# mbrzus/Cross-Modality-Minipig-Gan

Measured on AMD Instinct MI355X. Metric: T1->T2 256x256 slices/sec (G+D step), higher is better.
Workload: dtype f32

## Files before the change

cross-modality-minipig-gan_amd/_lib.py:

```python
from __future__ import annotations

import ctypes as C
import os

_HERE = os.path.dirname(os.path.abspath(__file__))
LIB_PATH = os.environ.get("MPGAN_LIB_PATH") or os.path.join(_HERE, "libmpgan_hip.so")
_lib = None


class ConvGeomC(C.Structure):
    _fields_ = [("n", C.c_int32), ("in_dhw", C.c_int32 * 3), ("out_dhw", C.c_int32 * 3),
                ("cin", C.c_int32), ("cout", C.c_int32), ("k", C.c_int32 * 3),
                ("stride", C.c_int32 * 3), ("pad", C.c_int32 * 3), ("transposed", C.c_int32),
                ("flags", C.c_int32), ("min_blocks", C.c_int32)]


class PeerTapsC(C.Structure):
    _fields_ = [("z_peer", C.c_void_p), ("ld_peer", C.c_int32), ("scale_peer", C.c_void_p),
                ("shift_peer", C.c_void_p), ("coef", C.c_void_p)]


class PeerTapsBF16C(C.Structure):
    _fields_ = [("z_peer", C.c_void_p), ("ld_peer", C.c_int32), ("scale_peer", C.c_void_p),
                ("shift_peer", C.c_void_p), ("coef", C.c_void_p)]
# ... 41 lines not shown
    "mpgan_conv_backward_data_stats_bf16": (_I, [_G, _P, _I, _P, _P, _I, _P, _I, _P, _P, _P, _P, _F, _P, _P]),
    "mpgan_conv_backward_data_stats": (_I, [_G, _P, _I, _P, _P, _I, _P, _I, _P, _P, _P, _P, _I, _F, _P, _P]),
    "mpgan_conv_wgrad_workspace": (_L, [_G]),
    "mpgan_conv_backward_weight": (_I, [_G, _P, _I, _PR, _P, _I, _P, _P, _F, _P, _L, _P]),
    "mpgan_conv_wgrad_kernel_name": (_I, [_G, _I, _I, C.c_char_p, _I]),
    "mpgan_pack_weights": (_I, [_P, _P, _P, _I, _L, _P]),
    "mpgan_stats_chunks": (_I, [_L, _I]),
    "mpgan_channel_stats": (_I, [_P, _I, _I, _L, _I, _P, _P]),
    "mpgan_norm_finalize": (_I, [_P, _I, _I, _I, _L, _I, _P, _P, _F, _F, _P, _P, _P, _P, _P, _P, _P, _P]),
    "mpgan_norm_finalize_strided": (_I, [_P, _I, _I, _I, _I, _L, _I, _P, _P, _F, _F, _P, _P, _P, _P, _P, _P, _P, _P]),
    "mpgan_norm_from_running": (_I, [_P, _P, _P, _P, _F, _I, _P, _P, _P, _P, _P]),
    "mpgan_norm_from_running_multi": (_I, [_P, _I, _P]),
    "mpgan_epi_vectors_multi": (_I, [_P, _I, _P]),
    "mpgan_conv_forward_act": (_I, [_G, _P, _I, _P, _P, _P, _P, _P, _I, _I, _P, _I, _P]),
    "mpgan_norm_act_add": (_I, [_P, _I, _PR, _P, _I, _PR, _I, _L, _I, _I, _P, _I, _P]),
    "mpgan_norm_bwd_reduce": (_I, [_P, _I, _P, _I, _PR, _P, _P, C.POINTER(PeerTapsC), _I, _L, _I, _P, _P]),
    "mpgan_tap_l1_partials": (_I, []),
    "mpgan_tap_l1": (_I, [_P, _I, _PR, _P, _I, _PR, _L, _I, _P, _P, _P]),
    "mpgan_conv_splitk_workspace": (_L, [_G]),
    "mpgan_conv_forward_splitk": (_I, [_G, _P, _I, _P, _P, _PR, _P, _L, _P, _I, _P]),
    "mpgan_sigmoid_forward": (_I, [_P, _I, _P, _P]),
    "mpgan_norm_bwd_finalize": (_I, [_P, _I, _I, _I, _L, _I, _P, _P, _P, _P, _P, _P]),
    "mpgan_norm_bwd_apply": (_I, [_P, _I, _P, _I, _PR, _P, _P, _P, _P, C.POINTER(PeerTapsC), _I, _L, _I, _P, _I, _P]),
    "mpgan_reduce_partials": (_I, [_P, _I, _I, _I, _P, _F, _P]),
    "mpgan_add_tanh": (_I, [_P, _P, _L, _I, _P, _P]),
    "mpgan_tanh_backward": (_I, [_P, _P, _L, _P, _P]),
    "mpgan_axpby": (_I, [_P, _F, _P, _F, _L, _P, _P]),
    "mpgan_copy_slice": (_I, [_P, _I, _P, _I, _L, _I, _I, _P]),
    "mpgan_linear1_partials": (_I, [_I]),
    "mpgan_linear1_forward": (_I, [_P, _PR, _I, _L, _I, _P, _P, _P, _P, _P, _P]),
    "mpgan_bce_forward": (_I, [_P, _P, _I, _P, _P]),
    "mpgan_bce_backward": (_I, [_P, _P, _I, _P, _P, _P]),
    "mpgan_sigmoid_backward": (_I, [_P, _P, _I, _P, _P]),
    "mpgan_scale_by_device_scalar": (_I, [_P, _P, _L, _P, _P]),
    "mpgan_weighted_sum": (_I, [_P, _P, _I, _P, _P]),
    "mpgan_debug_stamps": (_I, [_P, _L, _L]),
    "mpgan_debug_stamps_used": (_L, []),
    "mpgan_debug_clock_khz": (_I, []),
    "mpgan_linear1_backward": (_I, [_P, _PR, _I, _L, _I, _P, _P, _P, _P, _P, _F, _P]),
    "mpgan_sigmoid_bce": (_I, [_P, _I, _F, _F, _P, _P, _P, _P]),
    "mpgan_l1_partials": (_I, []),
    "mpgan_l1_loss": (_I, [_P, _P, _L, _F, _P, _P, _P, _P]),
    "mpgan_metric_partials": (_I, []),
    "mpgan_rescale_minmax": (_I, [_P, _L, _F, _F, _I, _P, _P, _P, _P]),
    "mpgan_image_errors": (_I, [_P, _P, _L, _F, _P, _P, _P]),
    "mpgan_percentile_workspace": (_L, []),
# ... 76 lines not shown
```

cross-modality-minipig-gan_amd/csrc/norm_ops.hip:

```cpp
#include "mpgan_common.h"
#include "norm_fold.h"

namespace mpgan {

static inline int stats_chunks_host(long pixels_per_sample, int C = 0) {
  long rows = 256;
  if (C >= 4 && C % 4 == 0) {
    long R = 256 / (C / 4);
    if (R < 1) R = 1;
    rows = 4 * R;
    if (rows > 256) rows = 256;
    if (rows < 16) rows = 16;
  }
  long c = pixels_per_sample / rows;
  if (c < 1) c = 1;
  if (c > 256) c = 256;
  return (int)c;
}

template <int V>
struct Vec;
template <>
struct Vec<4> {
  using T = float4;
// ... 514 lines not shown
      if (!ok[u]) continue;
      const long row = (long)n * P + pix0 + u * stride;
      float o[V];
#pragma unroll
      for (int e = 0; e < V; ++e) {
        const float y = zv[u][e] * sc[e] + sh[e];
        const float zh = (zv[u][e] - mu[e]) * is[e];
        float ga = gv[u][e], gy_extra = 0.f, dz_extra = 0.f;
        if (pr.coef) {
          const float yp = zp[u][e] * psc[e] + psh[e];
          const float ap = (leaky && yp < 0.f) ? yp * slope : yp;
          const float a = (leaky && y < 0.f) ? y * slope : y;
          ga -= ca * sgn(ap - a);
          gy_extra = -cy * sgn(yp - y);
          dz_extra = -cz * sgn(zp[u][e] - zv[u][e]);
        }
        const float gy = ((leaky && y < 0.f) ? ga * slope : ga) + gy_extra;
        o[e] = sc[e] * (gy - k1[e] - zh * k2[e]) + dz_extra;
      }
      Vec<V>::store(dz + row * lddz + c, o);
    }
  }
  (void)rows;
}

__global__ __launch_bounds__(256) void tap_l1_kernel(const float* __restrict__ za, int lda, Pro pa,
                                                     const float* __restrict__ zb, int ldb, Pro pb, long rows, int C,
                                                     float* __restrict__ partials) {
  __shared__ float sh[3][4];
  const float sa = pro_slope(pa), sb = pro_slope(pb);
  float s0 = 0.f, s1 = 0.f, s2 = 0.f;
  const long total = rows * C;
  for (long i = (long)blockIdx.x * blockDim.x + threadIdx.x; i < total; i += (long)gridDim.x * blockDim.x) {
    const long row = i / C;
    const int c = (int)(i - row * C);
    const float z1 = za[row * lda + c], z2 = zb[row * ldb + c];
    const float y1 = z1 * pa.scale[c] + pa.shift[c], y2 = z2 * pb.scale[c] + pb.shift[c];
    const float a1 = act_apply(y1, pa.act, sa), a2 = act_apply(y2, pb.act, sb);
    s0 += fabsf(z1 - z2);
    s1 += fabsf(y1 - y2);
    s2 += fabsf(a1 - a2);
  }
  s0 = wave_sum(s0); s1 = wave_sum(s1); s2 = wave_sum(s2);
  const int lane = threadIdx.x & 63, w = threadIdx.x >> 6;
  if (lane == 0) { sh[0][w] = s0; sh[1][w] = s1; sh[2][w] = s2; }
  __syncthreads();
// ... 226 lines not shown
                      ldg >= c && ldz >= c && lddz >= c,
                  "norm_bwd_apply: bad argument");
  const bool vec = (c % 4 == 0) && (ldz % 4 == 0) && (ldg % 4 == 0) && (lddz % 4 == 0) && aligned16(z) &&
                   aligned16(g) && aligned16(dz);
  const long rows = (long)n * P;
  Pro pp = make_pro(p);
  Peer pe = make_peer(peer);
  const int CGa = vec ? c / 4 : c;
  MPGAN_UNSUPPORTED(CGa > 256, "norm_bwd_apply: C=%d too wide", c);
  const int Ra = 256 / CGa;
  long gxa = (P + 4L * Ra - 1) / (4L * Ra);
  const long capa = 4096 / n > 1 ? 4096 / n : 1;
  if (gxa > capa) gxa = capa;
  dim3 grida((unsigned)gxa, (unsigned)n);
  if (vec)
    hipLaunchKernelGGL(norm_bwd_apply_kernel<4>, grida, dim3(256), 0, (hipStream_t)stream, g, ldg, z, ldz, pp, mean,
                       invstd, c1, c2, pe, rows, (long)P, c, dz, lddz);
  else
    hipLaunchKernelGGL(norm_bwd_apply_kernel<1>, grida, dim3(256), 0, (hipStream_t)stream, g, ldg, z, ldz, pp, mean,
                       invstd, c1, c2, pe, rows, (long)P, c, dz, lddz);
  return check_launch("norm_bwd_apply");
}

extern "C" int mpgan_reduce_partials(const float* partials, int32_t rows, int32_t row_stride, int32_t c, float* out,
                                     float beta, void* stream) {
  MPGAN_CHECK_ARG(partials && out && rows > 0 && c > 0 && row_stride >= c, "reduce_partials: bad argument");
  hipLaunchKernelGGL(reduce_partials_kernel, dim3((c + 3) / 4), dim3(256), 0, (hipStream_t)stream, partials, rows,
                     row_stride, c, out, beta);
  return check_launch("reduce_partials");
}

extern "C" int mpgan_copy_slice(const float* src, int32_t lds_, float* dst, int32_t ldd, int64_t pixels, int32_t c,
                                int32_t accumulate, void* stream) {
  MPGAN_CHECK_ARG(src && dst && pixels > 0 && c > 0 && lds_ >= c && ldd >= c, "copy_slice: bad argument");
  const bool vec = (c % 4 == 0) && (lds_ % 4 == 0) && (ldd % 4 == 0) && aligned16(src) && aligned16(dst);
  if (vec)
    hipLaunchKernelGGL(copy_slice_kernel<4>, dim3(ew_blocks(pixels * (c / 4))), dim3(256), 0, (hipStream_t)stream, src,
                       lds_, dst, ldd, (long)pixels, c, accumulate);
  else
    hipLaunchKernelGGL(copy_slice_kernel<1>, dim3(ew_blocks(pixels * c)), dim3(256), 0, (hipStream_t)stream, src, lds_,
                       dst, ldd, (long)pixels, c, accumulate);
  return check_launch("copy_slice");
}

__global__ void norm_from_running_kernel(const float* __restrict__ gamma, const float* __restrict__ beta,
                                         const float* __restrict__ rm, const float* __restrict__ rv, float eps, int c,
// ... 104 lines not shown
```

cross-modality-minipig-gan_amd/engine.py:

```python
from __future__ import annotations

import ctypes as C
import dataclasses
import math
import os
from typing import List, Optional, Sequence, Tuple

import torch
import torch.nn as nn

from . import ops
from ._lib import lib
from .ops import ACT_LEAKY, ACT_NONE, ConvGeom, Prologue


class KernelProbe:

    def __init__(self, want=None, detail=False, min_flops=0.0):
        self.want = want
        self.detail = detail
        self.min_flops = min_flops
        self.samples = []

    def summary(self):
# ... 438 lines not shown
                 C.byref(pc) if pc is not None else None, _p(resid), _ld(resid), int(tanh), _p(stats), y.data_ptr(),
                 _ld(y), keep=(gc, pc, x, wp, bias, y, resid, pro), desc=_gdesc(g), tag=tag, lane=lane)
        return
    assert stats is None or stats_acc is None
    prog.add("conv_forward_fold", lib().mpgan_conv_forward_fold, C.byref(gc), x.data_ptr(), _ld(x), wp.data_ptr(),
             _p(bias), C.byref(pc) if pc is not None else None, C.byref(fold) if fold is not None else None, _p(resid),
             _ld(resid), int(tanh), _p(stats), _p(stats_acc), ops.ACC_REPLICAS if stats_acc is not None else 0,
             y.data_ptr(), _ld(y), keep=(gc, pc, fold, x, wp, bias, y, resid, pro, stats_acc), desc=_gdesc(g), tag=tag,
             lane=lane)


def emit_conv_dgrad(prog, g: ConvGeom, dy, wp_bwd, dx, resid=None):
    ops._check_in_out(g, dx, dy, "plan conv_backward_data")
    gc = g.c()
    prog.add("conv_backward_data", lib().mpgan_conv_backward_data, C.byref(gc), dy.data_ptr(), _ld(dy),
             wp_bwd.data_ptr(), _p(resid), _ld(resid), dx.data_ptr(), _ld(dx), keep=(gc, dy, wp_bwd, dx, resid),
             desc=_gdesc(g), tag=("dgrad:" + gather_kernel_name(g, True, False), 2.0 * conv_macs(g), conv_bytes(g)))


_FUSE_BWD_STATS = not os.environ.get("MPGAN_DBG_NO_FUSE_BWD_STATS")
_FUSE_BWD_STATS_BF16 = bool(os.environ.get("MPGAN_FUSE_BWD_STATS_BF16"))


def emit_conv_dgrad_stats(prog, g: ConvGeom, dy, wp_bwd, dx, z, nb: "NormBuf", slope: float, partials) -> int:
    rows = ops.conv_bwd_stats_rows(g) if _FUSE_BWD_STATS and not nb.instance else 0
    if not rows or partials.numel() < rows * 3 * g.cin:
        emit_conv_dgrad(prog, g, dy, wp_bwd, dx)
        return 0
    ops._check_in_out(g, dx, dy, "plan conv_backward_data_stats")
    gc = g.c()
    prog.add("conv_backward_data", lib().mpgan_conv_backward_data_stats, C.byref(gc), dy.data_ptr(), _ld(dy),
             wp_bwd.data_ptr(), dx.data_ptr(), _ld(dx), z.data_ptr(), _ld(z), nb.scale.data_ptr(), nb.shift.data_ptr(),
             nb.mean.data_ptr(), nb.invstd.data_ptr(), ACT_LEAKY, float(slope), partials.data_ptr(),
             keep=(gc, dy, wp_bwd, dx, z, nb, partials), desc=_gdesc(g),
             tag=("dgrad:" + gather_kernel_name(g, True, False), 2.0 * conv_macs(g), conv_bytes(g)))
    return rows


def emit_conv_wgrad(prog, g: ConvGeom, x, dy, dw, ws, pro=None, dbias=None, lane=0):
    ops._check_in_out(g, x, dy, "plan conv_backward_weight")
    gc = g.c()
    pc = pro.c() if pro is not None else None
    need = ops.conv_wgrad_workspace(g)
    assert ws.numel() * 4 >= need, "wgrad workspace too small"
    prog.add("conv_backward_weight", lib().mpgan_conv_backward_weight, C.byref(gc), x.data_ptr(), _ld(x),
             C.byref(pc) if pc is not None else None, dy.data_ptr(), _ld(dy), dw.data_ptr(), _p(dbias), 1.0,
# ... 164 lines not shown
                 tag=_thin_cin1_tag(g, x))
        return
    prog.add("conv_forward_act_bf16", lib().mpgan_conv_forward_act_bf16, C.byref(gc), x.data_ptr(), g.cin, wp.data_ptr(),
             vec[0].data_ptr(), vec[1].data_ptr(), vec[2].data_ptr(), None, y.data_ptr(), g.cout,
             int(y.dtype == torch.float32), keep=(gc, x, wp, y, vec, norm_mod, act_mod, bias), desc=_gdesc(g),
             tag=(_bf16_kernel_name(g, False), 2.0 * conv_macs(g), conv_bytes(g, 2)))


def emit_norm_act_add(prog, z, pz, r, pr, out, tanh=False, fold=None):
    n, P, ldz = ops._cl(z, "norm_act_add z")
    assert out.shape == z.shape and (r is None or r.shape == z.shape)
    pzc = pz.c() if pz is not None else None
    prc = pr.c() if pr is not None else None
    if fold is None:
        prog.add("norm_act_add", lib().mpgan_norm_act_add, z.data_ptr(), ldz, C.byref(pzc) if pzc else None, _p(r),
                 _ld(r), C.byref(prc) if prc else None, n, P, z.shape[-1], int(tanh), out.data_ptr(), _ld(out),
                 keep=(z, pzc, pz, r, prc, pr, out), desc=f"C{z.shape[-1]} n{n} P{P}")
        return
    prog.add("norm_act_add_fold", lib().mpgan_norm_act_add_fold, z.data_ptr(), ldz, C.byref(pzc), C.byref(fold), _p(r),
             _ld(r), C.byref(prc) if prc else None, n, P, z.shape[-1], int(tanh), out.data_ptr(), _ld(out),
             keep=(z, pzc, pz, fold, r, prc, pr, out))


def emit_norm_bwd(prog, g, z, nb: NormBuf, pro: Prologue, dz, partials, dgamma, dbeta, dslope, peer=None, reduced_rows=0):
    n, P, ldz = ops._cl(z, "norm_bwd z")
    assert g.shape == z.shape and dz.shape == z.shape
    c = z.shape[-1]
    chunks = ops.stats_chunks(P, c)
    assert partials.numel() >= n * chunks * (3 * c + 1)
    L = lib()
    pc = pro.c()
    pe = peer.c() if peer is not None else None
    pe_ref = C.byref(pe) if pe is not None else None
    if reduced_rows:
        assert peer is None and not nb.instance and partials.numel() >= reduced_rows * 3 * c
        assert dslope is None, "fused norm-backward rows cannot feed a slope gradient"
        prog.add("norm_bwd_finalize", L.mpgan_norm_bwd_finalize, partials.data_ptr(), 1, reduced_rows, c, n * P, 0,
                 _p(dgamma), _p(dbeta), _p(dslope), nb.c1.data_ptr(), nb.c2.data_ptr(), keep=(dgamma, dbeta, dslope))
        prog.add("norm_bwd_apply", L.mpgan_norm_bwd_apply, g.data_ptr(), _ld(g), z.data_ptr(), ldz, C.byref(pc),
                 nb.mean.data_ptr(), nb.invstd.data_ptr(), nb.c1.data_ptr(), nb.c2.data_ptr(), pe_ref, n, P, c,
                 dz.data_ptr(), _ld(dz), keep=(dz, g, z, pc, pro, nb, partials), desc=f"C{c} n{n} P{P}")
        return
    prog.add("norm_bwd_reduce", L.mpgan_norm_bwd_reduce, g.data_ptr(), _ld(g), z.data_ptr(), ldz, C.byref(pc),
             nb.mean.data_ptr(), nb.invstd.data_ptr(), pe_ref, n, P, c, partials.data_ptr(),
             keep=(g, z, pc, pro, nb, partials, pe, peer), desc=f"C{c} n{n} P{P}")
    prog.add("norm_bwd_finalize", L.mpgan_norm_bwd_finalize, partials.data_ptr(), n, chunks, c, P, int(nb.instance),
             _p(dgamma), _p(dbeta), _p(dslope), nb.c1.data_ptr(), nb.c2.data_ptr(), keep=(dgamma, dbeta, dslope),
             desc=f"C{c} rows{n * chunks}")
    prog.add("norm_bwd_apply", L.mpgan_norm_bwd_apply, g.data_ptr(), _ld(g), z.data_ptr(), ldz, C.byref(pc),
             nb.mean.data_ptr(), nb.invstd.data_ptr(), nb.c1.data_ptr(), nb.c2.data_ptr(), pe_ref, n, P, c,
             dz.data_ptr(), _ld(dz), keep=(dz,), desc=f"C{c} n{n} P{P}")


def _bf16_kernel_name(g: ConvGeom, backward_data: bool) -> str:
    gc = g.c()
    return kernel_label(lib().mpgan_conv_kernel_name_bf16, C.byref(gc), int(backward_data))


def _bf16_wgrad_kernel_name(g: ConvGeom) -> str:
    gc = g.c()
    return "wgrad_bf16_wide_kernel" if lib().mpgan_conv_wgrad_variant_bf16(C.byref(gc)) == 1 else "wgrad_bf16_kernel<8>"


def _thin_cin1_tag(g: ConvGeom, x):
    return ("thin_cin1_full_kernel<16, true>", 2.0 * conv_macs(g), conv_bytes(g, 2) + 2 * x.numel())


def _rows(g: ConvGeom) -> int:
    return g.n * math.prod(g.out_dhw)


class PacksBF16:

    def __init__(self, recs, dev):
# ... 130 lines not shown
    def __exit__(self, *a):
        _GEOM_DEFAULTS.clear()
        _GEOM_DEFAULTS.update(self.saved)
        return False


def conv_geom_of(mod, n, in_dhw, dims) -> ConvGeom:
    tr = isinstance(mod, (nn.ConvTranspose2d, nn.ConvTranspose3d))
    k, s, p = _t3(mod.kernel_size, dims, 1), _t3(mod.stride, dims, 1), _t3(mod.padding, dims, 0)
    op = _t3(mod.output_padding, dims, 0) if tr else (0, 0, 0)
    return ConvGeom(n, tuple(in_dhw), mod.in_channels, mod.out_channels, k, s, p, tr, op, **_GEOM_DEFAULTS)


class Scratch:

    def __init__(self, dev):
        self.dev = dev
        self.partials_need = 0
        self.ws_need = 0
        self.partials = None
        self.ws = None

    def want_partials(self, n, P, c):
        self.partials_need = max(self.partials_need, (n * ops.stats_chunks(P, c) + 32) * (3 * c + 1) + c)

    def want_ws(self, g: ConvGeom):
        self.ws_need = max(self.ws_need, ops.conv_wgrad_workspace(g) // 4)
        rows = max(ops.conv_stats_rows(g, code) for code in (0, 1, 2))
        self.partials_need = max(self.partials_need, (rows + 32) * 2 * g.cout)

    def want_bf16_layer(self, g: ConvGeom, fused_rows=0):
        c, rows = g.cout, _rows(g)
        fwd_rows = (rows + 255) // 256 if g.cin == 1 else ops.conv_stats_rows_bf16(g)
        bwd_rows = max(ops.norm_bwd_rows_bf16(rows, c), fused_rows)
        self.partials_need = max(self.partials_need, (fwd_rows + 32) * 2 * c, (bwd_rows * 4 + 1) * c)
        ws = ops.conv_wgrad_workspace_bf16dy(g) if g.cin == 1 else ops.conv_wgrad_workspace_bf16(g)
        self.ws_need = max(self.ws_need, ws // 4)

    def alloc(self):
        self.partials = torch.empty(max(self.partials_need, 4), device=self.dev)
        self.ws = torch.empty(max(self.ws_need, 4), device=self.dev)


class _RU:

    def __init__(self, ru):
        self.units = []
# ... 255 lines not shown
            return

        own_mark, wait_mark = self._marks
        bw = Program()
        if wait_mark is not None:
            b.wait(wait_mark)
        G = a["gbufs"]
        gv = store.grad_view
        g_out, g_x = G["g_out"], G["g_x"]
        for l in range(0, L - 1):
            u = up_state[l]
            pt = prelu_pro(u["nbt"], u["AT"])
            g_u = g_out if l == 0 else G["gcat"][l - 1][..., chans[l - 1]:]
            if "zu" in u:
                dzu, gta = G["dzu"][l], G["gta"][l]
                emit_norm_bwd(b, g_u, u["zu"], u["nbu"], prelu_pro(u["nbu"], u["AU"]), dzu, part,
                              gv(u["NU"].weight), gv(u["NU"].bias), gv(u["AU"].weight))
                emit_conv_wgrad(bw, u["gu"], u["zt"], dzu, gv(u["cu"].weight), ws, pro=pt, dbias=gv(u["cu"].bias), lane=1)
                emit_conv_dgrad(b, u["gu"], dzu, wpb(R(u["cu"])), gta, resid=g_u)
            else:
                gta = G["gta"][l]
                emit_conv_wgrad(bw, u["gu"], u["ua"], g_u, gv(u["cu"].weight), ws, dbias=gv(u["cu"].bias), lane=1)
                emit_conv_dgrad(b, u["gu"], g_u, wpb(R(u["cu"])), gta, resid=g_u)
            emit_norm_bwd(b, gta, u["zt"], u["nbt"], pt, gta, part, gv(u["NT"].weight), gv(u["NT"].bias),
                          gv(u["AT"].weight))
            emit_bias_grad(b, gta, gv(u["ct"].bias), part)
            emit_conv_wgrad(bw, u["gt"], cats[l], gta, gv(u["ct"].weight), ws, lane=1)
            emit_conv_dgrad(b, u["gt"], gta, wpb(R(u["ct"])), G["gcat"][l])
        gcat_last = G["gcat"][L - 2]
        g_b = gcat_last[..., bt["cb_in"]:]
        gd_last = gcat_last[..., :bt["cb_in"]]
        d_last = cats[L - 2][..., :bt["cb_in"]]
        dzb1, gab0 = G["dzb1"], G["gab0"]
        emit_norm_bwd(b, g_b, bt["zb1"], bt["nbb1"], prelu_pro(bt["nbb1"], bt["BA1"]), dzb1, part,
                      gv(bt["BN1"].weight), gv(bt["BN1"].bias), gv(bt["BA1"].weight))
        emit_conv_wgrad(bw, bt["gb1"], bt["zb0"], dzb1, gv(bt["bc1"].weight), ws, pro=prelu_pro(bt["nbb0"], bt["BA0"]),
                        dbias=gv(bt["bc1"].bias), lane=1)
        emit_conv_dgrad(b, bt["gb1"], dzb1, wpb(R(bt["bc1"])), gab0)
        emit_norm_bwd(b, gab0, bt["zb0"], bt["nbb0"], prelu_pro(bt["nbb0"], bt["BA0"]), gab0, part,
                      gv(bt["BN0"].weight), gv(bt["BN0"].bias), gv(bt["BA0"].weight))
        emit_conv_wgrad(bw, bt["gb0"], d_last, gab0, gv(bt["bc0"].weight), ws, dbias=gv(bt["bc0"].bias), lane=1)
        emit_conv_dgrad(b, bt["gb0"], gab0, wpb(R(bt["bc0"])), gd_last, resid=gd_last)
        if bt["res"] is not None:
            emit_conv_wgrad(bw, bt["gbr"], d_last, g_b, gv(bt["res"].weight), ws, dbias=gv(bt["res"].bias), lane=1)
            emit_conv_dgrad(b, bt["gbr"], g_b, wpb(R(bt["res"])), gd_last, resid=gd_last)
        else:
            emit_norm_act_add(b, g_b, None, gd_last, None, gd_last)
        for l in range(L - 2, -1, -1):
            s = down_state[l]
            (cv0, N0, A0), (cv1, N1, A1) = s["ru"].units
            g_d = G["gcat"][l][..., :s["c"]]
            dz1, ga0 = G["dz1"][l], G["ga0"][l]
            emit_norm_bwd(b, g_d, s["z1"], s["nb1"], prelu_pro(s["nb1"], A1), dz1, part, gv(N1.weight), gv(N1.bias),
                          gv(A1.weight))
            emit_conv_wgrad(bw, s["g1"], s["z0"], dz1, gv(cv1.weight), ws, pro=prelu_pro(s["nb0"], A0),
                            dbias=gv(cv1.bias), lane=1)
            emit_conv_dgrad(b, s["g1"], dz1, wpb(R(cv1)), ga0)
            emit_norm_bwd(b, ga0, s["z0"], s["nb0"], prelu_pro(s["nb0"], A0), ga0, part, gv(N0.weight), gv(N0.bias),
                          gv(A0.weight))
            emit_conv_wgrad(bw, s["g0"], s["xin"], ga0, gv(cv0.weight), ws, dbias=gv(cv0.bias), lane=1)
            emit_conv_wgrad(bw, s["gr"], s["xin"], g_d, gv(s["ru"].res.weight), ws, dbias=gv(s["ru"].res.bias), lane=1)
            if l > 0:
                tgt = G["gcat"][l - 1][..., :chans[l - 1]]
                emit_conv_dgrad(b, s["g0"], ga0, wpb(R(cv0)), tgt, resid=tgt)
                emit_conv_dgrad(b, s["gr"], g_d, wpb(R(s["ru"].res)), tgt, resid=tgt)
            elif g_x is not None:
                emit_conv_dgrad(b, s["g0"], ga0, wpb(R(cv0)), g_x)
                emit_conv_dgrad(b, s["gr"], g_d, wpb(R(s["ru"].res)), g_x, resid=g_x)
        b.extend(bw)
        if own_mark is not None:
# ... 706 lines not shown
```

cross-modality-minipig-gan_amd/ops.py:

```python
from __future__ import annotations

import ctypes as C
import dataclasses
from dataclasses import dataclass
from typing import Optional, Sequence, Tuple

import torch

from ._lib import ConvGeomC, NormFoldC, PeerTapsBF16C, PeerTapsC, PrologueC, check, lib

ACT_NONE = 0
ACT_LEAKY = 1


def _stream() -> int:
    return torch.cuda.current_stream().cuda_stream


def _ptr(t: Optional[torch.Tensor]) -> Optional[int]:
    return None if t is None else t.data_ptr()


def _clx(t: torch.Tensor, dtype, what: str) -> Tuple[int, int, int]:
    if t.dim() != 5 or t.dtype != dtype or not t.is_cuda:
        raise ValueError(f"{what}: need a CUDA {dtype} (N,D,H,W,C) tensor, got {tuple(t.shape)} {t.dtype} {t.device}")
    n, d, h, w, c = t.shape
    st = t.stride()
    ld = st[3] if w > 1 else (st[2] if h > 1 else (st[1] if d > 1 else (st[0] if n > 1 else c)))
# ... 289 lines not shown
        raise ValueError("norm_bwd_reduce: partials too small (need n*chunks*(3*c + 1) floats)")
    check(lib().mpgan_norm_bwd_reduce(g.data_ptr(), ldg, z.data_ptr(), ldz, _pro(p), mean.data_ptr(),
                                      invstd.data_ptr(), _peer(peer), n, P, c, partials.data_ptr(), _stream()),
          "norm_bwd_reduce")


def norm_bwd_finalize(partials, n, chunks, c, P, instance, dgamma, dbeta, dslope, c1, c2):
    check(lib().mpgan_norm_bwd_finalize(partials.data_ptr(), n, chunks, c, P, int(instance), _ptr(dgamma), _ptr(dbeta),
                                        _ptr(dslope), c1.data_ptr(), c2.data_ptr(), _stream()), "norm_bwd_finalize")


def norm_bwd_apply(g, z, p: Prologue, mean, invstd, c1, c2, dz, peer: Optional[PeerTaps] = None):
    n, P, ldz = _cl(z, "norm_bwd_apply z")
    _, _, ldg = _cl(g, "norm_bwd_apply g")
    _, _, lddz = _cl(dz, "norm_bwd_apply dz")
    if g.shape != z.shape or dz.shape != z.shape:
        raise ValueError("norm_bwd_apply: shape mismatch")
    check(lib().mpgan_norm_bwd_apply(g.data_ptr(), ldg, z.data_ptr(), ldz, _pro(p), mean.data_ptr(),
                                     invstd.data_ptr(), c1.data_ptr(), c2.data_ptr(), _peer(peer), n, P, z.shape[-1],
                                     dz.data_ptr(), lddz, _stream()), "norm_bwd_apply")
    return dz


def tap_l1_partials() -> int:
    return int(lib().mpgan_tap_l1_partials())


def tap_l1(za, pa: Prologue, zb, pb: Prologue, partials, out3):
    n, P, lda = _cl(za, "tap_l1 a")
    _, _, ldb = _cl(zb, "tap_l1 b")
    if za.shape != zb.shape:
        raise ValueError("tap_l1: shape mismatch")
    check(lib().mpgan_tap_l1(za.data_ptr(), lda, _pro(pa), zb.data_ptr(), ldb, _pro(pb), n * P, za.shape[-1],
                             partials.data_ptr(), out3.data_ptr(), _stream()), "tap_l1")
    return out3


def conv_splitk_workspace(g: ConvGeom) -> int:
    gc = g.c()
    return int(lib().mpgan_conv_splitk_workspace(C.byref(gc)))


def conv_forward_splitk(g: ConvGeom, x, w_packed, bias, y, workspace, *, pro: Optional[Prologue] = None):
    _check_in_out(g, x, y, "conv_forward_splitk")
    _, _, ldx = _cl(x, "conv_forward_splitk x")
    _, _, ldy = _cl(y, "conv_forward_splitk y")
# ... 478 lines not shown
```

include/mpgan_hip.h:

```cpp
#ifndef MPGAN_HIP_H
#define MPGAN_HIP_H

#include <stdint.h>

#ifdef __cplusplus
extern "C" {
#endif

#define MPGAN_OK 0
#define MPGAN_ERR_INVALID -1
#define MPGAN_ERR_UNSUPPORTED -2
#define MPGAN_ERR_HIP -3

#define MPGAN_ACT_NONE 0
#define MPGAN_ACT_LEAKY 1

const char* mpgan_last_error(void);
int mpgan_abi_version(void);

typedef struct {
  int32_t n;
  int32_t in_dhw[3];
  int32_t out_dhw[3];
  int32_t cin, cout;
// ... 99 lines not shown

int mpgan_epi_vectors_multi(const int64_t* table, int32_t n_layers, void* stream);

int mpgan_norm_act_add(const float* z, int32_t ldz, const mpgan_prologue* pz,
                       const float* r, int32_t ldr, const mpgan_prologue* pr,
                       int32_t n, int64_t pixels_per_sample, int32_t c, int32_t tanh_out,
                       float* out, int32_t ldo, void* stream);

int mpgan_norm_bwd_reduce(const float* g, int32_t ldg, const float* z, int32_t ldz,
                          const mpgan_prologue* p, const float* mean, const float* invstd,
                          const mpgan_peer_taps* peer ,
                          int32_t n, int64_t pixels_per_sample, int32_t c,
                          float* partials, void* stream);
int mpgan_norm_bwd_finalize(const float* partials, int32_t n, int32_t chunks, int32_t c,
                            int64_t pixels_per_sample, int32_t instance,
                            float* dgamma, float* dbeta, float* dslope,
                            float* c1, float* c2, void* stream);
int mpgan_norm_bwd_apply(const float* g, int32_t ldg, const float* z, int32_t ldz,
                         const mpgan_prologue* p, const float* mean, const float* invstd,
                         const float* c1, const float* c2,
                         const mpgan_peer_taps* peer ,
                         int32_t n, int64_t pixels_per_sample, int32_t c,
                         float* dz, int32_t lddz, void* stream);

int mpgan_reduce_partials(const float* partials, int32_t rows, int32_t row_stride, int32_t c,
                          float* out, float beta, void* stream);

int mpgan_add_tanh(const float* a, const float* b, int64_t numel, int32_t apply_tanh,
                   float* y, void* stream);
int mpgan_tanh_backward(const float* g, const float* y, int64_t numel, float* dx, void* stream);
int mpgan_axpby(const float* a, float alpha, const float* b, float beta, int64_t numel,
                float* y, void* stream);
int mpgan_copy_slice(const float* src, int32_t lds, float* dst, int32_t ldd, int64_t pixels,
                     int32_t c, int32_t accumulate, void* stream);

int32_t mpgan_linear1_partials(int32_t n);
int mpgan_linear1_forward(const float* z, const mpgan_prologue* p, int32_t n,
                          int64_t pixels_per_sample, int32_t c, const float* w_perm,
                          const float* bias, float* partials, float* logit, float* prob ,
                          void* stream);
int mpgan_linear1_backward(const float* z, const mpgan_prologue* p, int32_t n,
                           int64_t pixels_per_sample, int32_t c, const float* w_perm,
                           const float* dlogit, float* g_a, float* dw, float* dbias,
                           float beta, void* stream);

int mpgan_sigmoid_bce(const float* logit, int32_t n, float target, float loss_scale,
// ... 200 lines not shown
```

Measured before the change: 294.6.

## Add folded BatchNorm backward kernels with fused bias grad and early wgrad flush

Adds an opt-in BatchNorm backward path. Reduction partials are folded per block and then finalized inside the apply kernel, which removes the separate finalize launch. The apply kernel also emits column sums so the conv bias gradient can be reduced without another pass over the gradient. Separately, the accumulated weight-gradient lane is flushed into the main backward program before the down-path loop by default. This changes the ordering and overlap of wgrad with dgrad work. The fold path is env-gated; the early wgrad reorder is active and may reduce or worsen overlap.

```diff
diff --git a/cross-modality-minipig-gan_amd/_lib.py b/cross-modality-minipig-gan_amd/_lib.py
--- a/cross-modality-minipig-gan_amd/_lib.py
+++ b/cross-modality-minipig-gan_amd/_lib.py
@@ -87,6 +87,9 @@
     "mpgan_sigmoid_forward": (_I, [_P, _I, _P, _P]),
     "mpgan_norm_bwd_finalize": (_I, [_P, _I, _I, _I, _L, _I, _P, _P, _P, _P, _P, _P]),
     "mpgan_norm_bwd_apply": (_I, [_P, _I, _P, _I, _PR, _P, _P, _P, _P, C.POINTER(PeerTapsC), _I, _L, _I, _P, _I, _P]),
+    "mpgan_norm_bwd_fold_rows": (_I, [_I, _L, _I, _P, _P, _P]),
+    "mpgan_norm_bwd_reduce_fold": (_I, [_P, _I, _P, _I, _PR, _P, _P, _I, _L, _I, _P, _P]),
+    "mpgan_norm_bwd_apply_fold": (_I, [_P, _I, _P, _I, _PR, _P, _P, _P, _I, _L, _I, _P, _P, _P, _P, _P, _P, _I, _P, _P]),
     "mpgan_reduce_partials": (_I, [_P, _I, _I, _I, _P, _F, _P]),
     "mpgan_add_tanh": (_I, [_P, _P, _L, _I, _P, _P]),
     "mpgan_tanh_backward": (_I, [_P, _P, _L, _P, _P]),
diff --git a/cross-modality-minipig-gan_amd/csrc/norm_ops.hip b/cross-modality-minipig-gan_amd/csrc/norm_ops.hip
--- a/cross-modality-minipig-gan_amd/csrc/norm_ops.hip
+++ b/cross-modality-minipig-gan_amd/csrc/norm_ops.hip
@@ -560,6 +560,225 @@
     }
   }
   (void)rows;
+}
+
+struct FoldLayout {
+  int rows, groups, Cg, adopt;
+};
+
+static inline FoldLayout fold_layout(int n, long P, int C) {
+  FoldLayout L;
+  L.groups = 1;
+  L.Cg = C;
+  if (C % 4 == 0)
+    while (L.Cg > 32 && L.Cg % 8 == 0) { L.Cg /= 2; L.groups *= 2; }
+  const long T = (long)n * P;
+  const int cgq = (C % 4 == 0) ? L.Cg / 4 : L.Cg;
+  const long R = cgq >= 256 ? 1 : 256 / cgq;
+  long rows = T / (4 * R);
+  const long cap = (48L * 1024 / 4) / (3L * C + L.groups);
+  if (rows > cap) rows = cap;
+  if (rows > 256) rows = 256;
+  if (rows < 1) rows = 1;
+  L.rows = (int)rows;
+  const bool vec_c = C % 4 == 0;
+  L.adopt = (C <= 128 && cap >= 1 && (vec_c || T * C <= (1L << 20))) ? 1 : 0;
+  return L;
+}
+
+static inline int fold_apply_blocks(int n, long P, int C) {
+  const int CG = (C % 4 == 0) ? C / 4 : C;
+  const long R = 256 / CG;
+  long b = ((long)n * P + 8 * R - 1) / (8 * R);
+  if (b > 256) b = 256;
+  if (b < 1) b = 1;
+  return (int)b;
+}
+
+template <int V>
+__global__ __launch_bounds__(256) void norm_bwd_reduce_fold_kernel(const float* __restrict__ gr, int ldg,
+                                                                   const float* __restrict__ z, int ldz, Pro p,
+                                                                   const float* __restrict__ mean,
+                                                                   const float* __restrict__ invstd, long T, int Cg,
+                                                                   float* __restrict__ partials) {
+  extern __shared__ float red[];
+  const float slope = pro_slope(p);
+  const bool leaky = p.act == MPGAN_ACT_LEAKY;
+  const int CGq = Cg / V, R = 256 / CGq;
+  const int tid = threadIdx.x;
+  const int q = tid % CGq, r = tid / CGq;
+  const int rows = gridDim.x, rb = blockIdx.x, grp = blockIdx.y;
+  const int cl = q * V, c = grp * Cg + cl;
+  const long per = (T + rows - 1) / rows;
+  const long beg = (long)rb * per;
+  const long end = beg + per < T ? beg + per : T;
+  float acc[3][V];
+#pragma unroll
+  for (int a = 0; a < 3; ++a)
+#pragma unroll
+    for (int e = 0; e < V; ++e) acc[a][e] = 0.f;
+  if (r < R) {
+    float sc[V], sh[V], mu[V], is[V];
+#pragma unroll
+    for (int e = 0; e < V; ++e) {
+      sc[e] = p.scale[c + e]; sh[e] = p.shift[c + e]; mu[e] = mean[c + e]; is[e] = invstd[c + e];
+    }
+    for (long pix0 = beg + r; pix0 < end; pix0 += 4L * R) {
+      float zv[4][V], gv[4][V];
+      bool ok[4];
+#pragma unroll
+      for (int u = 0; u < 4; ++u) {
+        const long pix = pix0 + (long)u * R;
+        ok[u] = pix < end;
+        const long row = ok[u] ? pix : pix0;
+        Vec<V>::load(z + row * ldz + c, zv[u]);
+        Vec<V>::load(gr + row * ldg + c, gv[u]);
+      }
+#pragma unroll
+      for (int u = 0; u < 4; ++u) {
+        if (!ok[u]) continue;
+#pragma unroll
+        for (int e = 0; e < V; ++e) {
+          const float y = zv[u][e] * sc[e] + sh[e];
+          const float zh = (zv[u][e] - mu[e]) * is[e];
+          const float ga = gv[u][e];
+          const bool neg = leaky && y < 0.f;
+          const float gy = neg ? ga * slope : ga;
+          acc[0][e] += gy;
+          acc[1][e] += gy * zh;
+          acc[2][e] += neg ? ga * y : 0.f;
+        }
+      }
+    }
+#pragma unroll
+    for (int a = 0; a < 3; ++a)
+#pragma unroll
+      for (int e = 0; e < V; ++e) red[(r * 3 + a) * Cg + cl + e] = acc[a][e];
+  }
+  __syncthreads();
+  const long rowi = (long)grp * rows + rb;
+  fold_rows(red, R, 3 * Cg, partials + rowi * 3 * Cg);
+  __syncthreads();
+  if (tid < 64) {
+    float t = 0.f;
+    for (int j = tid; j < Cg; j += 64) t += red[2 * Cg + j];
+    t = wave_sum(t);
+    if (tid == 0) partials[(long)gridDim.x * gridDim.y * 3 * Cg + rowi] = t;
+  }
+}
+
+template <int V>
+__global__ __launch_bounds__(256) void norm_bwd_apply_fold_kernel(const float* gr, int ldg, const float* __restrict__ z,
+                                                                  int ldz, Pro p, const float* __restrict__ mean,
+                                                                  const float* __restrict__ invstd,
+                                                                  const float* __restrict__ partials, int frows,
+                                                                  int groups, int Cg, double cnt, float* dgamma,
+                                                                  float* dbeta, float* dslope, float* c1, float* c2,
+                                                                  long T, int C, float* dz, int lddz,
+                                                                  float* __restrict__ colsum) {
+  __shared__ double fsum[256];
+  __shared__ float k1s[128], k2s[128];
+  __shared__ float cs[256 * V];
+  const int tid = threadIdx.x;
+  {
+    const int W = 2 * C;
+    int G = 1;
+    while (2 * G * W <= 256) G *= 2;
+    const int i = tid % W, gq = tid / W;
+    if (gq < G) {
+      const int qn = i / C, ch = i - qn * C;
+      const int grp = ch / Cg, cc = ch - grp * Cg;
+      const float* __restrict__ col = partials + ((long)grp * frows * 3 + qn) * Cg + cc;
+      double s = 0.0;
+      for (int r = gq; r < frows; r += 4 * G) {
+        float v[4];
+#pragma unroll
+        for (int u = 0; u < 4; ++u) {
+          const int rr = r + u * G;
+          v[u] = rr < frows ? col[(long)rr * 3 * Cg] : 0.f;
+        }
+#pragma unroll
+        for (int u = 0; u < 4; ++u) s += (double)v[u];
+      }
+      fsum[gq * W + i] = s;
+    }
+    __syncthreads();
+    for (int h = G >> 1; h > 0; h >>= 1) {
+      if (gq < h) fsum[gq * W + i] += fsum[(gq + h) * W + i];
+      __syncthreads();
+    }
+    if (tid < W) {
+      const double tot = fsum[tid];
+      const float k = (float)(tot / cnt);
+      if (tid < C) {
+        k1s[tid] = k;
+        if (blockIdx.x == 0) {
+          c1[tid] = k;
+          if (dbeta) dbeta[tid] += (float)tot;
+        }
+      } else {
+        k2s[tid - C] = k;
+        if (blockIdx.x == 0) {
+          c2[tid - C] = k;
+          if (dgamma) dgamma[tid - C] += (float)tot;
+        }
+      }
+    }
+    if (dslope && blockIdx.x == 0) slope_grad_block(partials + (long)frows * 3 * C, groups * frows, 0, dslope);
+    __syncthreads();
+  }
+  const int CG = C / V, R = 256 / CG;
+  const int q = tid % CG, r = tid / CG;
+  const int c = q * V;
+  const bool active = r < R;
+  float csum[V];
+#pragma unroll
+  for (int e = 0; e < V; ++e) csum[e] = 0.f;
+  if (active) {
+    const float slope = pro_slope(p);
+    const bool leaky = p.act == MPGAN_ACT_LEAKY;
+    float sc[V], sh[V], mu[V], is[V], k1[V], k2[V];
+#pragma unroll
+    for (int e = 0; e < V; ++e) {
+      sc[e] = p.scale[c + e]; sh[e] = p.shift[c + e]; mu[e] = mean[c + e]; is[e] = invstd[c + e];
+      k1[e] = k1s[c + e]; k2[e] = k2s[c + e];
+    }
+    const long stride = (long)gridDim.x * R;
+    for (long pix0 = (long)blockIdx.x * R + r; pix0 < T; pix0 += 4 * stride) {
+      float zv[4][V], gv[4][V];
+      bool ok[4];
+#pragma unroll
+      for (int u = 0; u < 4; ++u) {
+        const long pix = pix0 + u * stride;
+        ok[u] = pix < T;
+        const long row = ok[u] ? pix : pix0;
+        Vec<V>::load(z + row * ldz + c, zv[u]);
+        Vec<V>::load(gr + row * ldg + c, gv[u]);
+      }
+#pragma unroll
+      for (int u = 0; u < 4; ++u) {
+        if (!ok[u]) continue;
+        const long row = pix0 + u * stride;
+        float o[V];
+#pragma unroll
+        for (int e = 0; e < V; ++e) {
+          const float y = zv[u][e] * sc[e] + sh[e];
+          const float zh = (zv[u][e] - mu[e]) * is[e];
+          const float ga = gv[u][e];
+          const float gy = (leaky && y < 0.f) ? ga * slope : ga;
+          o[e] = sc[e] * (gy - k1[e] - zh * k2[e]);
+          csum[e] += o[e];
+        }
+        Vec<V>::store(dz + row * lddz + c, o);
+      }
+    }
+  }
+  if (!colsum) return;
+  if (active)
+#pragma unroll
+    for (int e = 0; e < V; ++e) cs[r * C + c + e] = csum[e];
+  __syncthreads();
+  fold_rows(cs, R, C, colsum + (long)blockIdx.x * C);
 }
 
 __global__ __launch_bounds__(256) void tap_l1_kernel(const float* __restrict__ za, int lda, Pro pa,
@@ -832,6 +1051,67 @@
   return check_launch("norm_bwd_apply");
 }
 
+extern "C" int32_t mpgan_norm_bwd_fold_rows(int32_t n, int64_t P, int32_t c, int32_t* groups, int32_t* apply_blocks,
+                                            int32_t* adopt) {
+  if (n <= 0 || P <= 0 || c <= 0) return 0;
+  const FoldLayout L = fold_layout(n, (long)P, c);
+  if (groups) *groups = L.groups;
+  if (apply_blocks) *apply_blocks = fold_apply_blocks(n, (long)P, c);
+  if (adopt) *adopt = L.adopt;
+  return L.rows;
+}
+
+extern "C" int mpgan_norm_bwd_reduce_fold(const float* g, int32_t ldg, const float* z, int32_t ldz,
+                                          const mpgan_prologue* p, const float* mean, const float* invstd, int32_t n,
+                                          int64_t P, int32_t c, float* partials, void* stream) {
+  MPGAN_CHECK_ARG(g && z && p && p->scale && mean && invstd && partials && n > 0 && P > 0 && c > 0 && ldg >= c &&
+                      ldz >= c,
+                  "norm_bwd_reduce_fold: bad argument");
+  MPGAN_UNSUPPORTED(p->n_stride != 0, "norm_bwd_reduce_fold: BatchNorm layers only (per-sample statistics given)");
+  const FoldLayout L = fold_layout(n, (long)P, c);
+  MPGAN_UNSUPPORTED(c > 128, "norm_bwd_reduce_fold: C=%d too wide", c);
+  const bool vec = (c % 4 == 0) && (ldz % 4 == 0) && (ldg % 4 == 0) && aligned16(z) && aligned16(g);
+  const int R = 256 / (vec ? L.Cg / 4 : L.Cg);
+  dim3 grid(L.rows, L.groups);
+  const size_t smem = (size_t)R * 3 * L.Cg * sizeof(float);
+  Pro pp = make_pro(p);
+  const long T = (long)n * P;
+  if (vec)
+    hipLaunchKernelGGL(norm_bwd_reduce_fold_kernel<4>, grid, dim3(256), smem, (hipStream_t)stream, g, ldg, z, ldz, pp,
+                       mean, invstd, T, L.Cg, partials);
+  else
+    hipLaunchKernelGGL(norm_bwd_reduce_fold_kernel<1>, grid, dim3(256), smem, (hipStream_t)stream, g, ldg, z, ldz, pp,
+                       mean, invstd, T, L.Cg, partials);
+  return check_launch("norm_bwd_reduce_fold");
+}
+
+extern "C" int mpgan_norm_bwd_apply_fold(const float* g, int32_t ldg, const float* z, int32_t ldz,
+                                         const mpgan_prologue* p, const float* mean, const float* invstd,
+                                         const float* partials, int32_t n, int64_t P, int32_t c, float* dgamma,
+                                         float* dbeta, float* dslope, float* c1, float* c2, float* dz, int32_t lddz,
+                                         float* colsum_partials, void* stream) {
+  MPGAN_CHECK_ARG(g && z && p && p->scale && mean && invstd && partials && c1 && c2 && dz && n > 0 && P > 0 && c > 0 &&
+                      ldg >= c && ldz >= c && lddz >= c,
+                  "norm_bwd_apply_fold: bad argument");
+  MPGAN_UNSUPPORTED(p->n_stride != 0, "norm_bwd_apply_fold: BatchNorm layers only (per-sample statistics given)");
+  const FoldLayout L = fold_layout(n, (long)P, c);
+  MPGAN_UNSUPPORTED(c > 128, "norm_bwd_apply_fold: C=%d too wide", c);
+  const bool vec = (c % 4 == 0) && (ldz % 4 == 0) && (ldg % 4 == 0) && (lddz % 4 == 0) && aligned16(z) &&
+                   aligned16(g) && aligned16(dz);
+  Pro pp = make_pro(p);
+  const long T = (long)n * P;
+  dim3 grida((unsigned)fold_apply_blocks(n, (long)P, c));
+  if (vec)
+    hipLaunchKernelGGL(norm_bwd_apply_fold_kernel<4>, grida, dim3(256), 0, (hipStream_t)stream, g, ldg, z, ldz, pp,
+                       mean, invstd, partials, L.rows, L.groups, L.Cg, (double)T, dgamma, dbeta, dslope, c1, c2, T, c,
+                       dz, lddz, colsum_partials);
+  else
+    hipLaunchKernelGGL(norm_bwd_apply_fold_kernel<1>, grida, dim3(256), 0, (hipStream_t)stream, g, ldg, z, ldz, pp,
+                       mean, invstd, partials, L.rows, L.groups, L.Cg, (double)T, dgamma, dbeta, dslope, c1, c2, T, c,
+                       dz, lddz, colsum_partials);
+  return check_launch("norm_bwd_apply_fold");
+}
+
 extern "C" int mpgan_reduce_partials(const float* partials, int32_t rows, int32_t row_stride, int32_t c, float* out,
                                      float beta, void* stream) {
   MPGAN_CHECK_ARG(partials && out && rows > 0 && c > 0 && row_stride >= c, "reduce_partials: bad argument");
diff --git a/cross-modality-minipig-gan_amd/engine.py b/cross-modality-minipig-gan_amd/engine.py
--- a/cross-modality-minipig-gan_amd/engine.py
+++ b/cross-modality-minipig-gan_amd/engine.py
@@ -484,6 +484,10 @@
 _FUSE_BWD_STATS_BF16 = bool(os.environ.get("MPGAN_FUSE_BWD_STATS_BF16"))
 
 
+_NORM_BWD_FOLD = bool(os.environ.get("MPGAN_NORM_BWD_FOLD"))
+_EARLY_WGRAD = not os.environ.get("MPGAN_DBG_LATE_WGRAD")
+
+
 def emit_conv_dgrad_stats(prog, g: ConvGeom, dy, wp_bwd, dx, z, nb: "NormBuf", slope: float, partials) -> int:
     rows = ops.conv_bwd_stats_rows(g) if _FUSE_BWD_STATS and not nb.instance else 0
     if not rows or partials.numel() < rows * 3 * g.cin:
@@ -694,10 +698,29 @@
              keep=(z, pzc, pz, fold, r, prc, pr, out))
 
 
-def emit_norm_bwd(prog, g, z, nb: NormBuf, pro: Prologue, dz, partials, dgamma, dbeta, dslope, peer=None, reduced_rows=0):
+def norm_bwd_folds(n, P, c, nb: "NormBuf", peer=None, reduced_rows=0) -> bool:
+    return bool(_NORM_BWD_FOLD and peer is None and not nb.instance and not reduced_rows
+                and ops.norm_bwd_fold_layout(n, P, c).adopt)
+
+
+def emit_norm_bwd(prog, g, z, nb: NormBuf, pro: Prologue, dz, partials, dgamma, dbeta, dslope, peer=None, reduced_rows=0,
+                  colsum=None) -> bool:
     n, P, ldz = ops._cl(z, "norm_bwd z")
     assert g.shape == z.shape and dz.shape == z.shape
     c = z.shape[-1]
+    if norm_bwd_folds(n, P, c, nb, peer, reduced_rows):
+        lay = ops.norm_bwd_fold_layout(n, P, c)
+        assert partials.numel() >= lay.partials(c) and not pro.n_stride
+        assert colsum is None or colsum.numel() >= lay.apply_blocks * c
+        L, pc = lib(), pro.c()
+        prog.add("norm_bwd_reduce_fold", L.mpgan_norm_bwd_reduce_fold, g.data_ptr(), _ld(g), z.data_ptr(), ldz,
+                 C.byref(pc), nb.mean.data_ptr(), nb.invstd.data_ptr(), n, P, c, partials.data_ptr(),
+                 keep=(g, z, pc, pro, nb, partials), desc=f"C{c} n{n} P{P}")
+        prog.add("norm_bwd_apply_fold", L.mpgan_norm_bwd_apply_fold, g.data_ptr(), _ld(g), z.data_ptr(), ldz,
+                 C.byref(pc), nb.mean.data_ptr(), nb.invstd.data_ptr(), partials.data_ptr(), n, P, c, _p(dgamma),
+                 _p(dbeta), _p(dslope), nb.c1.data_ptr(), nb.c2.data_ptr(), dz.data_ptr(), _ld(dz), _p(colsum),
+                 keep=(dz, dgamma, dbeta, dslope, colsum), desc=f"C{c} n{n} P{P} rows{lay.rows}x{lay.groups}")
+        return colsum is not None
     chunks = ops.stats_chunks(P, c)
     assert partials.numel() >= n * chunks * (3 * c + 1)
     L = lib()
@@ -712,7 +735,7 @@
         prog.add("norm_bwd_apply", L.mpgan_norm_bwd_apply, g.data_ptr(), _ld(g), z.data_ptr(), ldz, C.byref(pc),
                  nb.mean.data_ptr(), nb.invstd.data_ptr(), nb.c1.data_ptr(), nb.c2.data_ptr(), pe_ref, n, P, c,
                  dz.data_ptr(), _ld(dz), keep=(dz, g, z, pc, pro, nb, partials), desc=f"C{c} n{n} P{P}")
-        return
+        return False
     prog.add("norm_bwd_reduce", L.mpgan_norm_bwd_reduce, g.data_ptr(), _ld(g), z.data_ptr(), ldz, C.byref(pc),
              nb.mean.data_ptr(), nb.invstd.data_ptr(), pe_ref, n, P, c, partials.data_ptr(),
              keep=(g, z, pc, pro, nb, partials, pe, peer), desc=f"C{c} n{n} P{P}")
@@ -722,6 +745,7 @@
     prog.add("norm_bwd_apply", L.mpgan_norm_bwd_apply, g.data_ptr(), _ld(g), z.data_ptr(), ldz, C.byref(pc),
              nb.mean.data_ptr(), nb.invstd.data_ptr(), nb.c1.data_ptr(), nb.c2.data_ptr(), pe_ref, n, P, c,
              dz.data_ptr(), _ld(dz), keep=(dz,), desc=f"C{c} n{n} P{P}")
+    return False
 
 
 def _bf16_kernel_name(g: ConvGeom, backward_data: bool) -> str:
@@ -898,7 +922,8 @@
         self.ws = None
 
     def want_partials(self, n, P, c):
-        self.partials_need = max(self.partials_need, (n * ops.stats_chunks(P, c) + 32) * (3 * c + 1) + c)
+        self.partials_need = max(self.partials_need, (n * ops.stats_chunks(P, c) + 32) * (3 * c + 1) + c,
+                                 ops.norm_bwd_fold_layout(n, P, c).partials(c))
 
     def want_ws(self, g: ConvGeom):
         self.ws_need = max(self.ws_need, ops.conv_wgrad_workspace(g) // 4)
@@ -1200,9 +1225,18 @@
                 gta = G["gta"][l]
                 emit_conv_wgrad(bw, u["gu"], u["ua"], g_u, gv(u["cu"].weight), ws, dbias=gv(u["cu"].bias), lane=1)
                 emit_conv_dgrad(b, u["gu"], g_u, wpb(R(u["cu"])), gta, resid=g_u)
-            emit_norm_bwd(b, gta, u["zt"], u["nbt"], pt, gta, part, gv(u["NT"].weight), gv(u["NT"].bias),
-                          gv(u["AT"].weight))
-            emit_bias_grad(b, gta, gv(u["ct"].bias), part)
+            n_t, P_t, _ = ops._cl(gta, "bias grad")
+            bias_part = None
+            if norm_bwd_folds(n_t, P_t, u["co"], u["nbt"]):
+                bias_part = torch.empty(ops.norm_bwd_fold_layout(n_t, P_t, u["co"]).apply_blocks * u["co"],
+                                        device=gta.device)
+            if emit_norm_bwd(b, gta, u["zt"], u["nbt"], pt, gta, part, gv(u["NT"].weight), gv(u["NT"].bias),
+                             gv(u["AT"].weight), colsum=bias_part):
+                db = gv(u["ct"].bias)
+                bw.add("reduce_partials", lib().mpgan_reduce_partials, bias_part.data_ptr(),
+                       bias_part.numel() // u["co"], u["co"], u["co"], db.data_ptr(), 1.0, keep=(bias_part, db), lane=1)
+            else:
+                emit_bias_grad(b, gta, gv(u["ct"].bias), part)
             emit_conv_wgrad(bw, u["gt"], cats[l], gta, gv(u["ct"].weight), ws, lane=1)
             emit_conv_dgrad(b, u["gt"], gta, wpb(R(u["ct"])), G["gcat"][l])
         gcat_last = G["gcat"][L - 2]
@@ -1224,6 +1258,9 @@
             emit_conv_dgrad(b, bt["gbr"], g_b, wpb(R(bt["res"])), gd_last, resid=gd_last)
         else:
             emit_norm_act_add(b, g_b, None, gd_last, None, gd_last)
+        if _EARLY_WGRAD:
+            b.extend(bw)
+            bw = Program()
         for l in range(L - 2, -1, -1):
             s = down_state[l]
             (cv0, N0, A0), (cv1, N1, A1) = s["ru"].units
diff --git a/cross-modality-minipig-gan_amd/ops.py b/cross-modality-minipig-gan_amd/ops.py
--- a/cross-modality-minipig-gan_amd/ops.py
+++ b/cross-modality-minipig-gan_amd/ops.py
@@ -3,7 +3,7 @@
 import ctypes as C
 import dataclasses
 from dataclasses import dataclass
-from typing import Optional, Sequence, Tuple
+from typing import NamedTuple, Optional, Sequence, Tuple
 
 import torch
 
@@ -339,6 +339,56 @@
     return dz
 
 
+class FoldLayout(NamedTuple):
+    rows: int
+    groups: int
+    apply_blocks: int
+    adopt: bool
+
+    def partials(self, c: int) -> int:
+        return self.rows * (3 * c + self.groups)
+
+
+def norm_bwd_fold_layout(n: int, P: int, c: int) -> FoldLayout:
+    g, b, a = C.c_int32(0), C.c_int32(0), C.c_int32(0)
+    rows = int(lib().mpgan_norm_bwd_fold_rows(n, P, c, C.byref(g), C.byref(b), C.byref(a)))
+    if rows < 1:
+        raise ValueError(f"norm_bwd_fold_layout: bad shape n={n} P={P} c={c}")
+    return FoldLayout(rows, g.value, b.value, bool(a.value))
+
+
+def norm_bwd_reduce_fold(g, z, p: Prologue, mean, invstd, partials):
+    n, P, ldz = _cl(z, "norm_bwd_reduce_fold z")
+    _, _, ldg = _cl(g, "norm_bwd_reduce_fold g")
+    if g.shape != z.shape:
+        raise ValueError("norm_bwd_reduce_fold: shape mismatch")
+    c = z.shape[-1]
+    if partials.numel() < norm_bwd_fold_layout(n, P, c).partials(c):
+        raise ValueError("norm_bwd_reduce_fold: partials too small (need rows*(3*c + groups) floats)")
+    check(lib().mpgan_norm_bwd_reduce_fold(g.data_ptr(), ldg, z.data_ptr(), ldz, _pro(p), mean.data_ptr(),
+                                           invstd.data_ptr(), n, P, c, partials.data_ptr(), _stream()),
+          "norm_bwd_reduce_fold")
+
+
+def norm_bwd_apply_fold(g, z, p: Prologue, mean, invstd, partials, dgamma, dbeta, dslope, c1, c2, dz, colsum=None):
+    n, P, ldz = _cl(z, "norm_bwd_apply_fold z")
+    _, _, ldg = _cl(g, "norm_bwd_apply_fold g")
+    _, _, lddz = _cl(dz, "norm_bwd_apply_fold dz")
+    if g.shape != z.shape or dz.shape != z.shape:
+        raise ValueError("norm_bwd_apply_fold: shape mismatch")
+    c = z.shape[-1]
+    lay = norm_bwd_fold_layout(n, P, c)
+    if partials.numel() < lay.partials(c):
+        raise ValueError("norm_bwd_apply_fold: partials too small")
+    if colsum is not None and colsum.numel() < lay.apply_blocks * c:
+        raise ValueError("norm_bwd_apply_fold: colsum too small (need apply_blocks*c floats)")
+    check(lib().mpgan_norm_bwd_apply_fold(g.data_ptr(), ldg, z.data_ptr(), ldz, _pro(p), mean.data_ptr(),
+                                          invstd.data_ptr(), partials.data_ptr(), n, P, c, _ptr(dgamma), _ptr(dbeta),
+                                          _ptr(dslope), c1.data_ptr(), c2.data_ptr(), dz.data_ptr(), lddz,
+                                          _ptr(colsum), _stream()), "norm_bwd_apply_fold")
+    return dz
+
+
 def tap_l1_partials() -> int:
     return int(lib().mpgan_tap_l1_partials())
 
diff --git a/include/mpgan_hip.h b/include/mpgan_hip.h
--- a/include/mpgan_hip.h
+++ b/include/mpgan_hip.h
@@ -145,6 +145,18 @@
                          const mpgan_peer_taps* peer ,
                          int32_t n, int64_t pixels_per_sample, int32_t c,
                          float* dz, int32_t lddz, void* stream);
+
+int32_t mpgan_norm_bwd_fold_rows(int32_t n, int64_t pixels_per_sample, int32_t c, int32_t* groups,
+                                 int32_t* apply_blocks, int32_t* adopt);
+int mpgan_norm_bwd_reduce_fold(const float* g, int32_t ldg, const float* z, int32_t ldz,
+                               const mpgan_prologue* p, const float* mean, const float* invstd,
+                               int32_t n, int64_t pixels_per_sample, int32_t c,
+                               float* partials, void* stream);
+int mpgan_norm_bwd_apply_fold(const float* g, int32_t ldg, const float* z, int32_t ldz,
+                              const mpgan_prologue* p, const float* mean, const float* invstd,
+                              const float* partials, int32_t n, int64_t pixels_per_sample, int32_t c,
+                              float* dgamma, float* dbeta, float* dslope, float* c1, float* c2,
+                              float* dz, int32_t lddz, float* colsum_partials, void* stream);
 
 int mpgan_reduce_partials(const float* partials, int32_t rows, int32_t row_stride, int32_t c,
                           float* out, float beta, void* stream);
```

Result: no change. 296.0, median of 6 (+0.5%).
